# E3SM-Project/PAM

Measured on AMD Instinct MI355X. Metric: cell-updates/sec (AWFL dycore step), higher is better.
Workload: dtype f64; 1 GPU; AWFL supercell idealized, nens=1024/GPU, 32x32x60 L60, NT=1, fp64; scaling=weak, nens_total=1024, nens_per_gpu=1024, nx=32, ny=32, nz=60, num_tracers=1, parallelism=nens-shard x1, ranks_seen=1, limiter_input=0, fct_rows_flagged_last_stage=0, fct_rows=983040, lanes=member+xsweep

## Files before the change

### pam_amd/csrc/awfl_device.h

```cpp
#pragma once
#include <math.h>
#include <stdint.h>
#include <string.h>
#include <type_traits>
#include "awfl_constants.h"

#if defined(__HIPCC__)
#define PAMA_D __device__ __forceinline__
#else
#define PAMA_D inline
#endif

namespace pama {

constexpr int HS = 3;
constexpr int MAXT = 50;
constexpr int FLUX_THREADS = 256;
constexpr int FLUX_WAVES = FLUX_THREADS / 64;
#ifndef PAMA_FLUX_NF
#define PAMA_FLUX_NF 2
#endif
constexpr int FLUX_NF = PAMA_FLUX_NF;
constexpr int FLUX_MAX_SPAN = 64;
constexpr int VZ_STRIDE = 31;

enum PrimField { P_RHO = 0, P_PRES = 1, P_U = 2, P_V = 3, P_W = 4, P_THETA = 5, P_TR0 = 6 };

struct TracerPtrs { double *p[MAXT]; };

struct Params {
  int nens, nx, ny, nz, nt;
  int sim2d;
  int grav_balance;
  int vz_per_ens;
  int seg;
  int flat_cells;
  double dx, dy, rdx, rdy;
  double C0, gamma, grav, R_d, R_v;
  long long sx, sy, sz;
  long long prim_fs;
  long long ncell;
  long long fz_fs;
  const double *dz;
  const double *grav_var;
  const double *hy_dens;
  const double *hy_pres;
  const double *vz;
  const struct PowTab *pw;
  unsigned long long pos_mask, mass_mask;
  int idWV;
  int yz_fold;
  const double *rdz;
};

PAMA_D double fast_rcp(double x) {
#if defined(__HIP_DEVICE_COMPILE__)
  double y = __builtin_amdgcn_rcp(x);
  double r = fma(-x, y, 1.0);
  y = fma(y, r, y);
  r = fma(-x, y, 1.0);
  y = fma(y, r, y);
  return y;
#else
  return 1.0 / x;
#endif
}

PAMA_D double weno_rcp(double x) {
#if defined(__HIP_DEVICE_COMPILE__)
  double y = __builtin_amdgcn_rcp(x);
  double r = fma(-x, y, 1.0);
  return fma(y, r, y);
#else
  return 1.0 / x;
#endif
}

struct PowLog { double ic, lh, ll; };
struct PowExp { double th, tl; };
struct PowTab { PowLog lg[128]; PowExp ex[64]; };
struct PowLog2 { double hi, lo; };
PAMA_D PowLog2 pow_log2_dd(double x, const PowTab *T) {
#pragma clang fp contract(off)
  int e;
  double m = frexp(x, &e) * 2.0;
  e -= 1;
  unsigned long long bits;
#if defined(__HIP_DEVICE_COMPILE__)
  bits = (unsigned long long)__double_as_longlong(m);
#else
  memcpy(&bits, &m, 8);
#endif
  const int i = (int)((bits >> 45) & 127ull);
  const double ic = T->lg[i].ic, lh = T->lg[i].lh, ll = T->lg[i].ll;
  const double r = fma(m, ic, -1.0);
  const double Khi = 1.4426950408889634, Klo = 2.0355273740931033e-17;
  const double th = r * Khi;
  double tl = fma(r, Khi, -th);
  tl = fma(r, Klo, tl);
  double q = -0.18033688011112042;
  q = fma(q, r, 0.20609929155556620);
  q = fma(q, r, -0.24044917348149390);
  q = fma(q, r, 0.28853900817779268);
  q = fma(q, r, -0.36067376022224085);
  q = fma(q, r, 0.48089834696298783);
  q = fma(q, r, -0.72134752044448170);
  const double lo = fma(r * r, q, tl + ll);
  const double A = (double)e + lh;
  const double s = A + th, bb = s - A;
  const double err = (A - (s - bb)) + (th - bb);
  PowLog2 L;
  L.hi = s; L.lo = err + lo;
  return L;
}
PAMA_D double pow_exp2_dd(double x, double y, const PowLog2 L, const PowTab *T) {
#pragma clang fp contract(off)
  const double zh = y * L.hi;
  double zl = fma(y, L.hi, -zh);
  zl = fma(y, L.lo, zl);
  const double kd = rint(zh * 64.0);
  double f = fma(kd, -0.015625, zh);
  f += zl;
  double p = 1.5403530393381609e-4;
  p = fma(p, f, 1.3333558146428443e-3);
  p = fma(p, f, 9.6181291076284772e-3);
  p = fma(p, f, 5.5504108664821580e-2);
  p = fma(p, f, 2.4022650695910071e-1);
  p = fma(p, f, 6.9314718055994531e-1);
  p = p * f;
  if (!(x > 0.0)) return (x == 0.0) ? (y > 0.0 ? 0.0 : INFINITY) : NAN;
  if (!(x < INFINITY)) return y > 0.0 ? INFINITY : 0.0;
  const int k = (int)kd;
  const int j = k & 63, n = k >> 6;
  const double t2h = T->ex[j].th, t2l = T->ex[j].tl;
  return ldexp(fma(t2h, p, t2l) + t2h, n);
}
PAMA_D double pow_pos_fast(double x, double y, const PowTab *T) { return pow_exp2_dd(x, y, pow_log2_dd(x, T), T); }

PAMA_D double pow_pos(const Params &P, double x, double y) { return pow_pos_fast(x, y, P.pw); }

struct WenoConsts {
  double idl[4], sigma, ridl3;
  double c0[4], c1[4], c2[4], idl3x[4];
};
PAMA_D WenoConsts weno_consts() {
  WenoConsts w;
  const double raw[4] = AWFL_WENO_IDL_INIT;
  double sum = ((raw[0] + raw[1]) + raw[2]) + raw[3];
  for (int i = 0; i < 4; i++) w.idl[i] = raw[i] / (sum + 1.0e-20);
  w.sigma = AWFL_WENO_SIGMA;
  w.ridl3 = 1.0 / w.idl[3];
  for (int i = 0; i < 4; i++) {
    w.c0[i] = w.idl[i] + w.idl[i] * w.idl[i];
    w.c1[i] = 1.0 - 2.0 * w.idl[i];
    w.c2[i] = w.idl[i] * w.idl[i];
    w.idl3x[i] = 3.0 * w.idl[i];
  }
#if defined(__HIP_DEVICE_COMPILE__)
  asm("" : "+v"(w.idl3x[1]), "+v"(w.c0[1]), "+v"(w.c2[1]), "+v"(w.idl3x[3]), "+v"(w.c0[3]), "+v"(w.c2[3]));
  asm("" : "+v"(w.c2[0]));
  if (raw[0] == raw[2]) w.c2[2] = w.c2[0];
#endif
  return w;
}

struct WenoLin {
  double a1[3], a2[3];
  double h1, h2, h3, h4;
  double k2, k4, k2s;
};

constexpr double csqrt_(double v) {
  double x = v > 1.0 ? v : 1.0;
  for (int i = 0; i < 200; i++) x = 0.5 * (x + v / x);
  return x;
}
constexpr double WENO_K2U = 0.25 * AWFL_TV3_A2A2;
constexpr double WENO_SQRT_K2U = csqrt_(WENO_K2U), WENO_RSQRT_K2U = 1.0 / WENO_SQRT_K2U;
template <bool UNIFORM>
PAMA_D void weno5_blend(double u2, const WenoLin &p, const WenoConsts &wc, double &left, double &right) {
#pragma clang fp contract(off)
  constexpr double K13 = AWFL_TV5_A1A3 / AWFL_TV5_SQRT_A3A3, K24 = AWFL_TV5_A2A4 / AWFL_TV5_SQRT_A4A4;
  constexpr double EPS_TV = UNIFORM ? 1.0e-20 / (WENO_K2U * WENO_K2U) : 1.0e-20;
  constexpr double EPS_SUM = UNIFORM ? 1.0e-20 * (WENO_K2U * WENO_K2U) : 1.0e-20;
  constexpr double UNSCALE = UNIFORM ? WENO_SQRT_K2U : 1.0;
  double tv[4];
#pragma unroll
  for (int i = 0; i < 3; i++) {
    tv[i] = fma(p.a1[i], p.a1[i], p.a2[i] * p.a2[i]);
  }
  {
    const double t1 = fma(K13, p.h3, p.h1), t2 = fma(K24, p.h4, AWFL_TV5_A2A2 * p.h2);
    tv[3] = fma(p.h4, p.h4, fma(p.h3, p.h3, fma(p.h2, t2, p.h1 * t1)));
  }
  tv[3] = fma((1.0 - AWFL_WENO_SIGMA) / 3.0, (tv[0] + tv[1]) + tv[2], wc.sigma * tv[3]);
  const double d0 = fma(tv[0], tv[0], EPS_TV), d1 = fma(tv[1], tv[1], EPS_TV);
  const double d2 = fma(tv[2], tv[2], EPS_TV), d3 = fma(tv[3], tv[3], EPS_TV);
  const double p01 = d0 * d1, p23 = d2 * d3;
  const double x0 = d1 * p23, x1 = d0 * p23, x2 = d3 * p01, x3 = d2 * p01;
  const double n0 = wc.idl[0] * x0, n1 = wc.idl[1] * x1, n2 = wc.idl[2] * x2, n3 = wc.idl[3] * x3;
  const double rs = weno_rcp(fma(EPS_SUM, p01 * p23, fma(wc.idl[3], x3, fma(wc.idl[2], x2, fma(wc.idl[0], x0, n1)))));
  const double nn[4] = {n0, n1, n2, n3};
  double num[4], den[4];
#pragma unroll
  for (int i = 0; i < 4; i++) {
    const double w = nn[i] * rs;
    num[i] = w * fma(w, fma(nn[i], rs, -wc.idl3x[i]), wc.c0[i]);
    den[i] = fma(wc.c1[i], w, wc.c2[i]);
  }
  const double q01 = den[0] * den[1], q23 = den[2] * den[3];
  const double y0 = den[1] * q23, y1 = den[0] * q23, y2 = den[3] * q01, y3 = den[2] * q01;
  const double m0 = num[0] * y0, m1 = num[1] * y1, m2 = num[2] * y2, m3 = num[3] * y3;
  const double rm = weno_rcp(fma(num[3], y3, fma(num[2], y2, fma(num[1], y1, m0))));
  const double lo_e = fma(m0, p.a2[0], fma(m1, p.a2[1], m2 * p.a2[2]));
  double se;
  if (UNIFORM) se = fma(1.0 / 12.0, lo_e, m3 * fma(p.h4, UNSCALE * 0.05 / AWFL_TV5_SQRT_A4A4, p.h2 * (UNSCALE / 6.0)));
  else se = fma(p.k2s, lo_e, m3 * fma(p.h4, p.k4, p.h2 * p.k2));
  const double so = fma(m3, fma(0.25 / AWFL_TV5_SQRT_A3A3, p.h3, p.h1), fma(m0, p.a1[0], fma(m1, p.a1[1], m2 * p.a1[2])));
  const double even = fma(rm, se, u2);
  const double odd = ((0.5 * UNSCALE) * rm) * so;
  left = even - odd;
  right = even + odd;
}

struct DTable { double lo1[3][2], lo2[3][2], hi[4][4], k2, k4; };

constexpr double dcoef(const double c[5], int m) {
  return m == 1 ? -c[0] : m == 2 ? -c[0] - c[1] : m == 3 ? c[3] + c[4] : c[4];
}

constexpr DTable make_dtable(const double lo[3][3][3], const double hi[5][5], const double idl[4], double w) {
  DTable t{};
  double lod[3][3][4] = {};
  for (int i = 0; i < 3; i++)
    for (int ii = 0; ii < 3; ii++) {
      double c[5] = {0, 0, 0, 0, 0};
      for (int s = 0; s < 3; s++) c[i + s] = lo[i][s][ii];
      for (int m = 1; m <= 4; m++) lod[i][ii][m - 1] = dcoef(c, m);
    }
  double hid[5][4] = {};
  for (int ii = 0; ii < 5; ii++) {
    double c[5] = {hi[0][ii], hi[1][ii], hi[2][ii], hi[3][ii], hi[4][ii]};
    for (int m = 1; m <= 4; m++) {
      double v = dcoef(c, m);
      if (ii < 3)
        for (int i = 0; i < 3; i++) v -= idl[i] * lod[i][ii][m - 1];
      hid[ii][m - 1] = v / idl[3];
    }
  }
  for (int i = 0; i < 3; i++)
    for (int q = 0; q < 2; q++) {
      t.lo1[i][q] = lod[i][1][i + q];
      t.lo2[i][q] = lod[i][2][i + q];
    }
  for (int pp = 1; pp <= 4; pp++)
    for (int m = 0; m < 4; m++)
      t.hi[pp - 1][m] = hid[pp][m] * (pp == 3 ? AWFL_TV5_SQRT_A3A3 : (pp == 4 ? AWFL_TV5_SQRT_A4A4 : 1.0));
  t.k2 = 0.25 - w * w / 12.0;
  t.k4 = (0.0625 - w * w * w * w / 80.0) / AWFL_TV5_SQRT_A4A4;
  return t;
}

constexpr DTable make_const_dtable() {
  constexpr double S5[5][5] = AWFL_STEN_TO_COEFS_INIT;
  constexpr double W3[3][3][3] = AWFL_WENO_LOWER_INIT;
  constexpr double raw[4] = AWFL_WENO_IDL_INIT;
  double sum = ((raw[0] + raw[1]) + raw[2]) + raw[3];
  double idl[4] = {raw[0] / (sum + 1.0e-20), raw[1] / (sum + 1.0e-20), raw[2] / (sum + 1.0e-20), raw[3] / (sum + 1.0e-20)};
  return make_dtable(W3, S5, idl, 1.0);
}

constexpr double cabs_(double x) { return x < 0 ? -x : x; }
constexpr bool uniform_even_identity_holds() {
  constexpr double S5[5][5] = AWFL_STEN_TO_COEFS_INIT;
  constexpr double W3[3][3][3] = AWFL_WENO_LOWER_INIT;
  for (int i = 0; i < 3; i++)
    for (int s_ = 0; s_ < 3; s_++) {
      const double centre = (i + s_ == 2) ? 1.0 : 0.0;
      if (cabs_(W3[i][s_][0] + W3[i][s_][2] / 12.0 - centre) > 1e-15) return false;
    }
  for (int s_ = 0; s_ < 5; s_++) {
    const double centre = (s_ == 2) ? 1.0 : 0.0;
    if (cabs_(S5[s_][0] + S5[s_][2] / 12.0 + S5[s_][4] / 80.0 - centre) > 1e-15) return false;
  }
  return true;
}
static_assert(uniform_even_identity_holds(), "uniform-grid candidates must reproduce the centre cell average");

PAMA_D void weno5_const(const double u[5], const WenoConsts &wc, double &left, double &right) {
#pragma clang fp contract(off)
  constexpr DTable T = make_const_dtable();
  static_assert(T.hi[0][0] == T.hi[0][3] && T.hi[0][1] == T.hi[0][2], "x coefficient: symmetric");
  static_assert(T.hi[1][0] == -T.hi[1][3] && T.hi[1][1] == -T.hi[1][2], "x^2 coefficient: antisymmetric");
  static_assert(T.hi[2][0] == T.hi[2][3] && T.hi[2][1] == T.hi[2][2] && T.hi[2][0] == -T.hi[2][1], "x^3 coefficient");
  static_assert(T.hi[3][0] == -T.hi[3][3] && T.hi[3][1] == -T.hi[3][2] && cabs_(T.hi[3][1] + 3.0 * T.hi[3][0]) < 1e-14,
                "x^4 coefficient");
  static_assert(T.lo1[1][0] == 0.5 && T.lo1[1][1] == 0.5, "centred candidate slope");
  static_assert(T.lo2[0][0] == -0.5 && T.lo2[0][1] == 0.5 && T.lo2[1][0] == -0.5 && T.lo2[1][1] == 0.5 &&
                T.lo2[2][0] == -0.5 && T.lo2[2][1] == 0.5, "uniform-grid x^2 coefficients are half second differences");
  const double d[4] = {u[1] - u[0], u[2] - u[1], u[3] - u[2], u[4] - u[3]};
  WenoLin p;
  const double s03 = d[0] + d[3], s12 = d[1] + d[2], t03 = d[3] - d[0];
  p.a2[0] = d[1] - d[0];
  p.a2[1] = d[2] - d[1];
  p.a2[2] = d[3] - d[2];
  constexpr double S = WENO_RSQRT_K2U;
  p.a1[0] = fma(S * T.lo1[0][1], d[1], (S * T.lo1[0][0]) * d[0]);
  p.a1[1] = (S * 0.5) * s12;
  p.a1[2] = fma(S * T.lo1[2][1], d[3], (S * T.lo1[2][0]) * d[2]);
  p.h1 = fma(S * T.hi[0][1], s12, (S * T.hi[0][0]) * s03);
  p.h2 = fma(-S * T.hi[1][0], t03, (S * T.hi[1][2]) * p.a2[1]);
  p.h3 = (S * T.hi[2][0]) * (s03 - s12);
  p.h4 = (S * T.hi[3][3]) * fma(-3.0, p.a2[1], t03);
  p.k2 = p.k4 = p.k2s = 0.0;
  weno5_blend<true>(u[2], p, wc, left, right);
}

template <class TabPtr>
PAMA_D void weno5_table(const double u[5], TabPtr tab, long long ts, const WenoConsts &wc, double &left,
                        double &right) {
#pragma clang fp contract(off)
  const double d[4] = {u[1] - u[0], u[2] - u[1], u[3] - u[2], u[4] - u[3]};
  WenoLin p;
#pragma unroll
  for (int i = 0; i < 3; i++) {
    p.a1[i] = fma(tab[(1 + 2 * i) * ts], d[i + 1], tab[(0 + 2 * i) * ts] * d[i]);
    p.a2[i] = fma(tab[(7 + 2 * i) * ts], d[i + 1], tab[(6 + 2 * i) * ts] * d[i]);
  }
  p.h1 = fma(tab[12 * ts], d[0], fma(tab[13 * ts], d[1], fma(tab[14 * ts], d[2], tab[15 * ts] * d[3])));
  p.h2 = fma(tab[16 * ts], d[0], fma(tab[17 * ts], d[1], fma(tab[18 * ts], d[2], tab[19 * ts] * d[3])));
  p.h3 = fma(tab[20 * ts], d[0], fma(tab[21 * ts], d[1], fma(tab[22 * ts], d[2], tab[23 * ts] * d[3])));
  p.h4 = fma(tab[24 * ts], d[0], fma(tab[25 * ts], d[1], fma(tab[26 * ts], d[2], tab[27 * ts] * d[3])));
  p.k2 = tab[28 * ts];
  p.k4 = tab[29 * ts];
  p.k2s = tab[30 * ts];
  weno5_blend<false>(u[2], p, wc, left, right);
}

PAMA_D double mul_rn(double a, double b) {
#pragma clang fp contract(off)
  return a * b;
}

PAMA_D void acoustic_face(double ru_L, double ru_R, double pp_L, double pp_R, bool wall, double &ruf, double &ppf) {
#pragma clang fp contract(off)
  const double cs = 350.0, rcs = 1.0 / 350.0;
  if (wall) { ru_L = 0.0; ru_R = 0.0; }
  const double w1 = 0.5 * fma(-cs, ru_R, pp_R);
  const double w2 = 0.5 * fma(cs, ru_L, pp_L);
  ppf = w1 + w2;
  ruf = (w2 - w1) * rcs;
  if (wall) ruf = 0.0;
}

PAMA_D double flux_divergence(const Params &P, double xlo, double xhi, double ylo, double yhi, double zlo, double zhi,
                              double rdzk) {
#pragma clang fp contract(off)
  double tend = (xlo - xhi) * P.rdx;
  if (!P.sim2d) tend = fma(ylo - yhi, P.rdy, tend);
  return fma(zlo - zhi, rdzk, tend);
}

PAMA_D double yz_divergence(const Params &P, double dyv, double dzv, double rdzk) {
#pragma clang fp contract(off)
  return fma(dzv, rdzk, dyv * P.rdy);
}
PAMA_D double flux_divergence_g(const Params &P, double xlo, double xhi, double yz) {
#pragma clang fp contract(off)
  return fma(xlo - xhi, P.rdx, yz);
}
PAMA_D double flux_divergence_d(const Params &P, double xlo, double xhi, double dyv, double dzv, double rdzk) {
#pragma clang fp contract(off)
  if (P.sim2d) return fma(dzv, rdzk, (xlo - xhi) * P.rdx);
  return flux_divergence_g(P, xlo, xhi, yz_divergence(P, dyv, dzv, rdzk));
}

PAMA_D double gravity_coef(const Params &P, long long ke) { return P.grav_balance ? P.grav_var[ke] : P.hy_dens[ke]; }
PAMA_D double add_gravity(const Params &P, double tend, double rho_in, double gcoef) {
#pragma clang fp contract(off)
  if (P.grav_balance) return fma(-gcoef, rho_in, tend);
  return fma(-P.grav, rho_in - gcoef, tend);
}

template <int STAGE>
PAMA_D double rk_combine(double m_0, double m_in, double dt_dyn, double tend) {
#pragma clang fp contract(off)
  if (STAGE == 1) return fma(dt_dyn, tend, m_in);
  if (STAGE == 2) return fma((1.0 / 4.0) * dt_dyn, tend, fma(1.0 / 4.0, m_in, (3.0 / 4.0) * m_0));
  return fma((2.0 / 3.0) * dt_dyn, tend, fma(2.0 / 3.0, m_in, (1.0 / 3.0) * m_0));
}
template <int STAGE>
PAMA_D double next_seed(double m_0, double m_in, double v) {
#pragma clang fp contract(off)
  if (STAGE == 1) return fma(1.0 / 4.0, v, (3.0 / 4.0) * m_in);
  if (STAGE == 2) return fma(2.0 / 3.0, v, (1.0 / 3.0) * m_0);
  return v;
}

#if defined(__HIP_DEVICE_COMPILE__)
typedef const __attribute__((address_space(1))) double *gc_ptr;
typedef __attribute__((address_space(1))) double *g_ptr;
PAMA_D gc_ptr uni(const double *p) {
  const unsigned long long v = (unsigned long long)p;
  const unsigned lo = __builtin_amdgcn_readfirstlane((unsigned)v), hi = __builtin_amdgcn_readfirstlane((unsigned)(v >> 32));
  return (gc_ptr)(((unsigned long long)hi << 32) | lo);
}
PAMA_D g_ptr uniw(double *p) { return (g_ptr)uni(p); }
typedef const __attribute__((address_space(4))) double *const_ptr;
PAMA_D const_ptr as_constant(const double *p) { return (const_ptr)(unsigned long long)p; }
PAMA_D int uni_int(int v) {
  int r = __builtin_amdgcn_readfirstlane(v);
  asm volatile("" : "+s"(r));
  return r;
}
#else
typedef const double *gc_ptr;
typedef double *g_ptr;
PAMA_D gc_ptr uni(const double *p) { return p; }
PAMA_D g_ptr uniw(double *p) { return p; }
typedef const double *const_ptr;
PAMA_D const_ptr as_constant(const double *p) { return p; }
PAMA_D int uni_int(int v) { return v; }
#endif
PAMA_D unsigned member_offset(int e) { return (unsigned)e & 0x0fffffffu; }

PAMA_D void store_adv_u(const Params &P, double *prim, int pf, int k, long long cu, unsigned e, double val, double ghost_val) {
  double *f = prim + (long long)pf * P.prim_fs + cu;
  uniw(f + (long long)(k + HS) * P.sz)[e] = val;
  if (k == 0)
    for (int kk = 0; kk < HS; kk++) uniw(f + (long long)(HS - 1 - kk) * P.sz)[e] = ghost_val;
  if (k == P.nz - 1)
    for (int kk = 0; kk < HS; kk++) uniw(f + (long long)(HS + P.nz + kk) * P.sz)[e] = ghost_val;
}

struct LineGeom {
  int dir;
  int n;
  int nfaces;
  long long cs;
  long long fs_flux;
};

PAMA_D LineGeom line_geom(const Params &P, int dir) {
  LineGeom g;
  g.dir = dir;
  if (dir == 0) { g.n = P.nx; g.nfaces = P.nx; g.cs = P.sx; g.fs_flux = P.ncell; }
  else if (dir == 1) { g.n = P.ny; g.nfaces = P.ny; g.cs = P.sy; g.fs_flux = P.ncell; }
  else { g.n = P.nz; g.nfaces = P.nz + 1; g.cs = P.sz; g.fs_flux = P.fz_fs; }
  return g;
}

PAMA_D int wrap(int c, int n) {
  c %= n;
  return c < 0 ? c + n : c;
}

#if defined(__HIPCC__)
#define PAMA_HD __host__ __device__ inline
#else
#define PAMA_HD inline
#endif
PAMA_HD int further_tracer(const Params &P, int i) { return i < P.idWV ? i : i + 1; }
PAMA_HD bool skip_advected_v(const Params &P, bool diff) { return diff && P.sim2d; }
PAMA_HD int flux_sweep_pairs(const Params &P, bool diff) { return (3 + P.nt - (skip_advected_v(P, diff) ? 1 : 0) + 1) / 2; }

struct LineLane { long long pbase, fbase; unsigned eu; int et; };
template <int DIR>
PAMA_D LineLane member_lane(const Params &P, int line, int e) {
  LineLane ll;
  ll.eu = member_offset(e);
  ll.et = e;
  if (DIR == 0) {
    const int k = uni_int(line / P.ny), j = line - k * P.ny;
    ll.pbase = (long long)(k + HS) * P.sz + (long long)j * P.sy;
    ll.fbase = (long long)k * P.sz + (long long)j * P.sy;
  } else if (DIR == 1) {
    const int k = uni_int(line / P.nx), i = line - k * P.nx;
    ll.pbase = (long long)(k + HS) * P.sz + (long long)i * P.sx;
    ll.fbase = (long long)k * P.sz + (long long)i * P.sx;
  } else {
    ll.pbase = (long long)HS * P.sz + (long long)line * P.sx;
    ll.fbase = (long long)line * P.sx;
  }
  return ll;
}
PAMA_HD long long flat_items(const Params &P, int dir) { return (long long)(dir == 1 ? P.nz : P.ny) * P.nx * P.nens; }
template <int DIR>
PAMA_D LineLane flat_lane(const Params &P, unsigned q) {
  static_assert(DIR == 1 || DIR == 2, "flat lanes: y and z sweeps (the x direction has its own tile kernels)");
  LineLane ll;
  ll.pbase = (long long)HS * P.sz;
  ll.fbase = 0;
  const unsigned row = (unsigned)P.nx * (unsigned)P.nens;
  if (DIR == 1) {
    const unsigned k = q / row, r = q - k * row;
    ll.eu = member_offset((int)(k * (unsigned)P.sz + r));
    ll.et = (int)(r % (unsigned)P.nens);
  } else {
    ll.eu = member_offset((int)q);
    ll.et = (int)(q % (unsigned)P.nens);
  }
  return ll;
}

struct ZTabConst {
  const double *vz;
  PAMA_D double rdz(const Params &P, int k, int) const { return as_constant(P.rdz + (long long)k * P.nens)[0]; }
  PAMA_D void pass_begin(int, int) {}
  PAMA_D void trip_begin(int) {}
  PAMA_D void trip_end(int) {}
  PAMA_D void weno(const double u[5], int level, const WenoConsts &wc, double &L, double &R) const {
    weno5_table(u, as_constant(vz + (long long)level * VZ_STRIDE), 1, wc, L, R);
  }
};
struct ZTabLane {
  const double *vz;
  long long nens;
  int e;
  PAMA_D double rdz(const Params &P, int k, int e_) const { return P.rdz[(long long)k * P.nens + e_]; }
  PAMA_D void pass_begin(int, int) {}
  PAMA_D void trip_begin(int) {}
  PAMA_D void trip_end(int) {}
  PAMA_D void weno(const double u[5], int level, const WenoConsts &wc, double &L, double &R) const {
    weno5_table(u, vz + (long long)level * VZ_STRIDE * nens + e, nens, wc, L, R);
  }
};

template <int DIR, bool DIFF, class ZT, bool FOLD = false>
PAMA_D void flux_line_body_zt(const Params &P, const double *__restrict__ prim, double *__restrict__ flux, const LineLane &ll,
                              int f0, int span, int pair_sel, ZT &zt, const double *__restrict__ fold_y = nullptr) {
  static_assert(!FOLD || (DIR == 2 && DIFF), "only the z sweep of the fused stage folds the y differences in");
  const unsigned eu = ll.eu;
  const int e = ll.et;
  const LineGeom g = line_geom(P, DIR);
  const WenoConsts wc = weno_consts();
  const long long pbase = ll.pbase, fbase = ll.fbase;
  const int fend = (f0 + span < g.nfaces) ? f0 + span : g.nfaces;
  const int cl = DIFF ? (fend < g.n ? fend : g.n) : fend - 1;
  const bool periodic = (DIR != 2);
  const bool reuse0 = DIFF && periodic && f0 == 0 && cl == g.n;
  const int cloop = reuse0 ? cl - 1 : cl;
  const int ncomp = (DIR == 0) ? P_U : (DIR == 1 ? P_V : P_W);

  auto cell_off = [&](int c) -> long long {
    if (DIR == 2) return pbase + (long long)(c > P.nz + 2 ? P.nz + 2 : c) * g.cs;
    return pbase + (long long)(c < 0 ? c + g.n : (c >= g.n ? c - g.n : c)) * g.cs;
  };
  auto weno = [&](const double u[5], int c, double &L, double &R) {
    if (DIR != 2) { weno5_const(u, wc, L, R); return; }
    zt.weno(u, c + 1, wc, L, R);
  };
  auto fold_cell = [&](int c) -> int { return c > 0 ? c - 1 : 0; };
  auto folded = [&](double dzv, double dyv, double rdzv) -> double { return yz_divergence(P, dyv, dzv, rdzv); };
  const int nadv = 4 + P.nt;
  double *fl0 = flux + fbase;

  if (pair_sel <= 0) {
    const double *pr = prim + (long long)P_RHO * P.prim_fs;
    const double *pn = prim + (long long)ncomp * P.prim_fs;
    const double *pp = prim + (long long)P_PRES * P.prim_fs;
    double *fln = flux + (long long)(1 + ncomp - P_U) * g.fs_flux + fbase;
    double wm[5], wp[5], wn[5];
#pragma unroll
    for (int s = 0; s < 5; s++) {
      const long long o = cell_off(f0 - 3 + s);
      wn[s] = uni(pn + o)[eu];
      wm[s] = mul_rn(uni(pr + o)[eu], wn[s]);
      wp[s] = uni(pp + o)[eu];
    }
    double prevR_m, prevR_p, prevR_n;
    if (DIR == 2) { zt.pass_begin(f0, cloop + 1); zt.trip_begin(f0); }
    {
      double Lm, Lp, Ln;
      weno(wm, f0 - 1, Lm, prevR_m);
      weno(wp, f0 - 1, Lp, prevR_p);
      weno(wn, f0 - 1, Ln, prevR_n);
      const long long on = cell_off(f0 + 2);
      const double nn = uni(pn + on)[eu];
#pragma unroll
      for (int s = 0; s < 4; s++) { wm[s] = wm[s + 1]; wp[s] = wp[s + 1]; wn[s] = wn[s + 1]; }
      wn[4] = nn; wm[4] = mul_rn(uni(pr + on)[eu], nn); wp[4] = uni(pp + on)[eu];
    }
    if (DIR == 2) zt.trip_end(f0);
    double Fpn = 0.0, Fn0 = 0.0;
    const double *fyn = FOLD ? fold_y + (long long)(1 + ncomp - P_U) * P.ncell + fbase : nullptr;
#pragma clang loop unroll(disable)
    for (int c = f0; c <= cloop; c++) {
      if (DIR == 2) zt.trip_begin(c + 1);
      const long long on = cell_off(c + 3);
      const double nn = uni(pn + on)[eu], nm = mul_rn(uni(pr + on)[eu], nn), np_ = uni(pp + on)[eu];
      double dyv = 0.0, rdzv = 0.0;
      if (FOLD) {
        dyv = uni(fyn + (long long)fold_cell(c) * g.cs)[eu];
        rdzv = zt.rdz(P, fold_cell(c), e);
      }
      double Lm, Rm, Lp, Rp, Ln, Rn;
      weno(wm, c, Lm, Rm);
      weno(wp, c, Lp, Rp);
      weno(wn, c, Ln, Rn);
      const bool wall = (DIR == 2) && (c == 0 || c == P.nz);
      double ruf, ppf;
      acoustic_face(prevR_m, Lm, prevR_p, Lp, wall, ruf, ppf);
      const double val = (ruf > 0.0) ? prevR_n : Ln;
      const double fn = fma(ruf, val, ppf);
      if (!(DIFF && periodic && c == g.n)) uniw(fl0 + (long long)c * g.cs)[eu] = ruf;
      if (DIFF) {
        if (c > f0) uniw(fln + (long long)(c - 1) * g.cs)[eu] = FOLD ? folded(Fpn - fn, dyv, rdzv) : Fpn - fn;
        else Fn0 = fn;
        Fpn = fn;
      } else {
        uniw(fln + (long long)c * g.cs)[eu] = fn;
      }
      prevR_m = Rm; prevR_p = Rp; prevR_n = Rn;
#pragma unroll
      for (int s = 0; s < 4; s++) { wm[s] = wm[s + 1]; wp[s] = wp[s + 1]; wn[s] = wn[s + 1]; }
      wm[4] = nm; wp[4] = np_; wn[4] = nn;
      if (DIR == 2) zt.trip_end(c + 1);
    }
    if (reuse0) uniw(fln + (long long)(g.n - 1) * g.cs)[eu] = Fpn - Fn0;
  }
  auto sweep = [&](auto nf_tag, auto ns_tag, const int *fa) __attribute__((always_inline)) {
    constexpr int NF = decltype(nf_tag)::value;
    constexpr int NS = decltype(ns_tag)::value;
    const double *q[NF];
    double *fl[NF];
    double w[NF][5], prevR[NF];
#pragma unroll
    for (int n = 0; n < NF; n++) {
      q[n] = prim + (long long)(P_U + fa[n]) * P.prim_fs;
      fl[n] = flux + (long long)(1 + fa[n]) * g.fs_flux + fbase;
    }
#pragma unroll
    for (int s = 0; s < 5; s++) {
      const long long o = cell_off(f0 - 3 + s);
#pragma unroll
      for (int n = 0; n < NF; n++) w[n][s] = uni(q[n] + o)[eu];
    }
    if (DIR == 2) { zt.pass_begin(f0, cloop + 1); zt.trip_begin(f0); }
    {
// ... 1753 lines not shown
```

Before: 2.520 billion cell-updates/s.

## Fold WENO ideal weights into smoothness denominators and diagonalize uniform-grid TV form

Rewrites the WENO5 weight computation so the ideal weights are absorbed into the per-candidate denominators as constant ratios, which removes the per-cell multiplications by wc.idl. For uniform grids it precomputes at compile time a block-diagonalized quadratic form for the blended high-order total variation, so that value comes from a few squares of linear combinations of differences instead of building the h1..h4 coefficients. A shared tail function produces left and right directly with fmas. This cuts FLOPs in the hot reconstruction, but it changes the rounding order and relies on the ideal weights staying constant and matching the static_asserts.

```diff
diff --git a/pam_amd/csrc/awfl_device.h b/pam_amd/csrc/awfl_device.h
--- a/pam_amd/csrc/awfl_device.h
+++ b/pam_amd/csrc/awfl_device.h
@@ -177,50 +177,59 @@
 }
 constexpr double WENO_K2U = 0.25 * AWFL_TV3_A2A2;
 constexpr double WENO_SQRT_K2U = csqrt_(WENO_K2U), WENO_RSQRT_K2U = 1.0 / WENO_SQRT_K2U;
-template <bool UNIFORM>
-PAMA_D void weno5_blend(double u2, const WenoLin &p, const WenoConsts &wc, double &left, double &right) {
+constexpr double weno_idl_c(int i) {
+  constexpr double raw[4] = AWFL_WENO_IDL_INIT;
+  return raw[i] / ((((raw[0] + raw[1]) + raw[2]) + raw[3]) + 1.0e-20);
+}
+constexpr double WENO_R1 = weno_idl_c(0) / weno_idl_c(1), WENO_R3 = weno_idl_c(0) / weno_idl_c(3);
+static_assert(weno_idl_c(0) == weno_idl_c(2), "weights 0 and 2 share their ideal weight");
+constexpr double WENO_BLEND_LO = (1.0 - AWFL_WENO_SIGMA) / 3.0;
+
+PAMA_D void weno5_tail(double u2, double d0, double d1, double d2, double d3, double eps_sum, const double (&a1)[3],
+                       const double (&a2)[3], double e3, double o3, double kse, double codd, const WenoConsts &wc, double &left,
+                       double &right) {
 #pragma clang fp contract(off)
-  constexpr double K13 = AWFL_TV5_A1A3 / AWFL_TV5_SQRT_A3A3, K24 = AWFL_TV5_A2A4 / AWFL_TV5_SQRT_A4A4;
-  constexpr double EPS_TV = UNIFORM ? 1.0e-20 / (WENO_K2U * WENO_K2U) : 1.0e-20;
-  constexpr double EPS_SUM = UNIFORM ? 1.0e-20 * (WENO_K2U * WENO_K2U) : 1.0e-20;
-  constexpr double UNSCALE = UNIFORM ? WENO_SQRT_K2U : 1.0;
-  double tv[4];
-#pragma unroll
-  for (int i = 0; i < 3; i++) {
-    tv[i] = fma(p.a1[i], p.a1[i], p.a2[i] * p.a2[i]);
-  }
-  {
-    const double t1 = fma(K13, p.h3, p.h1), t2 = fma(K24, p.h4, AWFL_TV5_A2A2 * p.h2);
-    tv[3] = fma(p.h4, p.h4, fma(p.h3, p.h3, fma(p.h2, t2, p.h1 * t1)));
-  }
-  tv[3] = fma((1.0 - AWFL_WENO_SIGMA) / 3.0, (tv[0] + tv[1]) + tv[2], wc.sigma * tv[3]);
-  const double d0 = fma(tv[0], tv[0], EPS_TV), d1 = fma(tv[1], tv[1], EPS_TV);
-  const double d2 = fma(tv[2], tv[2], EPS_TV), d3 = fma(tv[3], tv[3], EPS_TV);
   const double p01 = d0 * d1, p23 = d2 * d3;
   const double x0 = d1 * p23, x1 = d0 * p23, x2 = d3 * p01, x3 = d2 * p01;
-  const double n0 = wc.idl[0] * x0, n1 = wc.idl[1] * x1, n2 = wc.idl[2] * x2, n3 = wc.idl[3] * x3;
-  const double rs = weno_rcp(fma(EPS_SUM, p01 * p23, fma(wc.idl[3], x3, fma(wc.idl[2], x2, fma(wc.idl[0], x0, n1)))));
-  const double nn[4] = {n0, n1, n2, n3};
+  const double rs = weno_rcp(fma(x3, fma(eps_sum, d3, 1.0), (x0 + x1) + x2));
+  const double xx[4] = {x0, x1, x2, x3};
   double num[4], den[4];
 #pragma unroll
   for (int i = 0; i < 4; i++) {
-    const double w = nn[i] * rs;
-    num[i] = w * fma(w, fma(nn[i], rs, -wc.idl3x[i]), wc.c0[i]);
+    const double w = xx[i] * rs;
+    num[i] = w * fma(w, fma(xx[i], rs, -wc.idl3x[i]), wc.c0[i]);
     den[i] = fma(wc.c1[i], w, wc.c2[i]);
   }
   const double q01 = den[0] * den[1], q23 = den[2] * den[3];
   const double y0 = den[1] * q23, y1 = den[0] * q23, y2 = den[3] * q01, y3 = den[2] * q01;
   const double m0 = num[0] * y0, m1 = num[1] * y1, m2 = num[2] * y2, m3 = num[3] * y3;
   const double rm = weno_rcp(fma(num[3], y3, fma(num[2], y2, fma(num[1], y1, m0))));
-  const double lo_e = fma(m0, p.a2[0], fma(m1, p.a2[1], m2 * p.a2[2]));
-  double se;
-  if (UNIFORM) se = fma(1.0 / 12.0, lo_e, m3 * fma(p.h4, UNSCALE * 0.05 / AWFL_TV5_SQRT_A4A4, p.h2 * (UNSCALE / 6.0)));
-  else se = fma(p.k2s, lo_e, m3 * fma(p.h4, p.k4, p.h2 * p.k2));
-  const double so = fma(m3, fma(0.25 / AWFL_TV5_SQRT_A3A3, p.h3, p.h1), fma(m0, p.a1[0], fma(m1, p.a1[1], m2 * p.a1[2])));
-  const double even = fma(rm, se, u2);
-  const double odd = ((0.5 * UNSCALE) * rm) * so;
-  left = even - odd;
-  right = even + odd;
+  const double lo_e = fma(m0, a2[0], fma(m1, a2[1], m2 * a2[2]));
+  const double se = fma(kse, lo_e, m3 * e3);
+  const double so = fma(m3, o3, fma(m0, a1[0], fma(m1, a1[1], m2 * a1[2])));
+  left = fma(rm, fma(-codd, so, se), u2);
+  right = fma(rm, fma(codd, so, se), u2);
+}
+
+PAMA_D void weno5_blend(double u2, const WenoLin &p, const WenoConsts &wc, double &left, double &right) {
+#pragma clang fp contract(off)
+  constexpr double K13 = AWFL_TV5_A1A3 / AWFL_TV5_SQRT_A3A3, K24 = AWFL_TV5_A2A4 / AWFL_TV5_SQRT_A4A4;
+  constexpr double EPS_TV = 1.0e-20;
+  double tv[4];
+#pragma unroll
+  for (int i = 0; i < 3; i++) {
+    tv[i] = fma(p.a1[i], p.a1[i], p.a2[i] * p.a2[i]);
+  }
+  {
+    const double t1 = fma(K13, p.h3, p.h1), t2 = fma(K24, p.h4, AWFL_TV5_A2A2 * p.h2);
+    tv[3] = fma(p.h4, p.h4, fma(p.h3, p.h3, fma(p.h2, t2, p.h1 * t1)));
+  }
+  const double tv3s = fma(WENO_BLEND_LO / AWFL_WENO_SIGMA, (tv[0] + tv[1]) + tv[2], tv[3]);
+  constexpr double R3S = WENO_R3 * (AWFL_WENO_SIGMA * AWFL_WENO_SIGMA);
+  const double d0 = fma(tv[0], tv[0], EPS_TV), d1 = fma(tv[1], tv[1] * WENO_R1, EPS_TV * WENO_R1);
+  const double d2 = fma(tv[2], tv[2], EPS_TV), d3 = fma(tv3s, tv3s * R3S, EPS_TV * WENO_R3);
+  weno5_tail(u2, d0, d1, d2, d3, 1.0e-20 / weno_idl_c(0), p.a1, p.a2, fma(p.h4, p.k4, p.h2 * p.k2),
+             fma(0.25 / AWFL_TV5_SQRT_A3A3, p.h3, p.h1), p.k2s, 0.5, wc, left, right);
 }
 
 struct DTable { double lo1[3][2], lo2[3][2], hi[4][4], k2, k4; };
@@ -286,6 +295,55 @@
   return true;
 }
 static_assert(uniform_even_identity_holds(), "uniform-grid candidates must reproduce the centre cell average");
+
+struct UniformUpper { double lam, a1, b1, a3, b3, eta, xt, xa, hs, hc, cross; };
+constexpr UniformUpper make_uniform_upper() {
+  constexpr DTable T = make_const_dtable();
+  constexpr double S = WENO_RSQRT_K2U, K13 = AWFL_TV5_A1A3 / AWFL_TV5_SQRT_A3A3, K24 = AWFL_TV5_A2A4 / AWFL_TV5_SQRT_A4A4;
+  double Q[4][4] = {};
+  for (int i = 0; i < 3; i++) {
+    double va[4] = {}, vb[4] = {};
+    va[i] = S * T.lo1[i][0]; va[i + 1] = S * T.lo1[i][1];
+    vb[i] = -1.0; vb[i + 1] = 1.0;
+    for (int r = 0; r < 4; r++)
+      for (int c = 0; c < 4; c++) Q[r][c] += WENO_BLEND_LO * (va[r] * va[c] + vb[r] * vb[c]);
+  }
+  double h[4][4] = {};
+  for (int q = 0; q < 4; q++)
+    for (int m = 0; m < 4; m++) h[q][m] = S * T.hi[q][m];
+  for (int r = 0; r < 4; r++)
+    for (int c = 0; c < 4; c++)
+      Q[r][c] += AWFL_WENO_SIGMA * (h[0][r] * h[0][c] + 0.5 * K13 * (h[0][r] * h[2][c] + h[2][r] * h[0][c]) +
+                                    AWFL_TV5_A2A2 * h[1][r] * h[1][c] + 0.5 * K24 * (h[1][r] * h[3][c] + h[3][r] * h[1][c]) +
+                                    h[2][r] * h[2][c] + h[3][r] * h[3][c]);
+  const double P[4][4] = {{0.5, 0, -0.5, 0}, {0, 0.5, 0, -0.5}, {0, 0.5, 0, 0.5}, {0.5, 0, 0.5, 0}};
+  double M[4][4] = {};
+  for (int r = 0; r < 4; r++)
+    for (int c = 0; c < 4; c++)
+      for (int a = 0; a < 4; a++)
+        for (int b = 0; b < 4; b++) M[r][c] += P[a][r] * Q[a][b] * P[b][c];
+  UniformUpper U{};
+  const double ce = M[1][1] - M[0][1] * M[0][1] / M[0][0], co = M[3][3] - M[2][3] * M[2][3] / M[2][2];
+  U.lam = 0.25 * S * S / ce;
+  U.a1 = csqrt_(U.lam * M[0][0]); U.b1 = U.lam * M[0][1] / U.a1;
+  U.a3 = csqrt_(U.lam * M[2][2]); U.b3 = U.lam * M[2][3] / U.a3;
+  U.eta = U.lam * co - 1.0;
+  double x[4] = {}, hh[4] = {};
+  for (int m = 0; m < 4; m++) {
+    x[m] = T.hi[1][m] / 6.0 + 0.05 * T.hi[3][m] / AWFL_TV5_SQRT_A4A4;
+    hh[m] = S * (T.hi[0][m] + 0.25 * T.hi[2][m] / AWFL_TV5_SQRT_A3A3);
+  }
+  U.xt = x[3]; U.xa = x[2];
+  U.hs = hh[0]; U.hc = hh[1];
+  for (int r = 0; r < 2; r++)
+    for (int c = 2; c < 4; c++) U.cross = cabs_(M[r][c]) > U.cross ? cabs_(M[r][c]) : U.cross;
+  return U;
+}
+constexpr bool uniform_upper_ok() {
+  constexpr UniformUpper U = make_uniform_upper();
+  return U.cross < 1e-15 && U.lam > 0.0 && U.eta > -1.0 && U.a1 > 0.0 && U.a3 > 0.0;
+}
+static_assert(uniform_upper_ok(), "uniform-grid blended TV: positive definite blocks");
 
 PAMA_D void weno5_const(const double u[5], const WenoConsts &wc, double &left, double &right) {
 #pragma clang fp contract(off)
@@ -298,22 +356,28 @@
   static_assert(T.lo1[1][0] == 0.5 && T.lo1[1][1] == 0.5, "centred candidate slope");
   static_assert(T.lo2[0][0] == -0.5 && T.lo2[0][1] == 0.5 && T.lo2[1][0] == -0.5 && T.lo2[1][1] == 0.5 &&
                 T.lo2[2][0] == -0.5 && T.lo2[2][1] == 0.5, "uniform-grid x^2 coefficients are half second differences");
+  constexpr UniformUpper U = make_uniform_upper();
+  constexpr double EPS_TV = 1.0e-20 / (WENO_K2U * WENO_K2U);
+  constexpr double EPS_SUM = 1.0e-20 * (WENO_K2U * WENO_K2U);
   const double d[4] = {u[1] - u[0], u[2] - u[1], u[3] - u[2], u[4] - u[3]};
-  WenoLin p;
   const double s03 = d[0] + d[3], s12 = d[1] + d[2], t03 = d[3] - d[0];
-  p.a2[0] = d[1] - d[0];
-  p.a2[1] = d[2] - d[1];
-  p.a2[2] = d[3] - d[2];
+  double a1[3], a2[3];
+  a2[0] = d[1] - d[0];
+  a2[1] = d[2] - d[1];
+  a2[2] = d[3] - d[2];
   constexpr double S = WENO_RSQRT_K2U;
-  p.a1[0] = fma(S * T.lo1[0][1], d[1], (S * T.lo1[0][0]) * d[0]);
-  p.a1[1] = (S * 0.5) * s12;
-  p.a1[2] = fma(S * T.lo1[2][1], d[3], (S * T.lo1[2][0]) * d[2]);
-  p.h1 = fma(S * T.hi[0][1], s12, (S * T.hi[0][0]) * s03);
-  p.h2 = fma(-S * T.hi[1][0], t03, (S * T.hi[1][2]) * p.a2[1]);
-  p.h3 = (S * T.hi[2][0]) * (s03 - s12);
-  p.h4 = (S * T.hi[3][3]) * fma(-3.0, p.a2[1], t03);
-  p.k2 = p.k4 = p.k2s = 0.0;
-  weno5_blend<true>(u[2], p, wc, left, right);
+  a1[0] = fma(S * T.lo1[0][1], d[1], (S * T.lo1[0][0]) * d[0]);
+  a1[1] = (S * 0.5) * s12;
+  a1[2] = fma(S * T.lo1[2][1], d[3], (S * T.lo1[2][0]) * d[2]);
+  const double sq1 = a2[1] * a2[1];
+  const double tv0 = fma(a1[0], a1[0], a2[0] * a2[0]), tv1 = fma(a1[1], a1[1], sq1), tv2 = fma(a1[2], a1[2], a2[2] * a2[2]);
+  const double l1 = fma(U.a1, s03, U.b1 * s12), l3 = fma(U.a3, t03, U.b3 * a2[1]);
+  const double tvb = fma(l1, l1, fma(l3, l3, fma(U.eta, sq1, tv1)));
+  constexpr double R3L = WENO_R3 / (U.lam * U.lam);
+  const double d0 = fma(tv0, tv0, EPS_TV), d1 = fma(tv1, tv1 * WENO_R1, EPS_TV * WENO_R1);
+  const double d2 = fma(tv2, tv2, EPS_TV), d3 = fma(tvb, tvb * R3L, EPS_TV * WENO_R3);
+  weno5_tail(u[2], d0, d1, d2, d3, EPS_SUM / weno_idl_c(0), a1, a2, fma(U.xt, t03, U.xa * a2[1]), fma(U.hs, s03, U.hc * s12),
+             1.0 / 12.0, 0.5 * WENO_SQRT_K2U, wc, left, right);
 }
 
 template <class TabPtr>
@@ -334,7 +398,7 @@
   p.k2 = tab[28 * ts];
   p.k4 = tab[29 * ts];
   p.k2s = tab[30 * ts];
-  weno5_blend<false>(u[2], p, wc, left, right);
+  weno5_blend(u[2], p, wc, left, right);
 }
 
 PAMA_D double mul_rn(double a, double b) {
```

Measured after the change: 2.623 billion cell-updates/s, median of 6. +4.1%, better.
